# kamalmostafa/minimodem

Hardware: NVIDIA B200
Metric: audio Msamples/s demodulated (batched streams) (higher is better)
Workload: dtype f32

## Files before the change

### minimodem_b200/csrc/fsk_b200_device.cuh

```cuda
#ifndef FSK_B200_DEVICE_CUH
#define FSK_B200_DEVICE_CUH

#include <cuda_runtime.h>
#include <stdint.h>

#include "fsk_b200_internal.h"

#define FSK_FLT_EPSILON 1.1920928955078125e-07f
#define ACC_BLOCK 64u
#define FAST_MAX_N 2048u


__device__ __forceinline__ bool decide_bit(float mag_mark, float mag_space, unsigned expect,
	float2 *slot)
{
    const bool one = mag_mark > mag_space;
    const float sig = one ? mag_mark : mag_space;
    const float noise = one ? mag_space : mag_mark;
    *slot = make_float2(sig, one ? -noise : noise);
    return expect != 2u && expect != (one ? 1u : 0u);
}

__device__ __forceinline__ bool needs_resum(float mag_mark, float mag_space)
{
// ... 162 lines not shown
    }
    return best_c;
}

template <int G, class Src>
__device__ __forceinline__ float find_frame(const Src &src, unsigned base,
	const fsk_b200_geom &geo, int sel, const float4 *__restrict__ tw, float2 *scr,
	unsigned g, unsigned gmask, unsigned try_first, unsigned try_max, unsigned try_step,
	float limit, unsigned long long &best_bits, float &best_a, unsigned &best_t)
{
    return search_frames([&](unsigned t, unsigned long long &bits, float &a) {
	return frame_analyze<G, Src>(src, base + t, geo, sel, tw, scr, g, gmask, bits, a);
    }, try_first, try_max, try_step, limit, best_bits, best_a, best_t);
}


struct Ring {
    unsigned ring_s;
    unsigned R, pad;
};

__device__ __forceinline__ unsigned ring_wrap(unsigned off, unsigned R) { return off >= R ? off - R : off; }

#ifndef FSK_EMU
__device__ __forceinline__ float fast_sqrt(float x)
{
    float r;
    asm("sqrt.approx.ftz.f32 %0, %1;" : "=f"(r) : "f"(x));
    return r;
}
__device__ __forceinline__ float fast_div(float a, float b)
{
    float r;
    asm("div.approx.ftz.f32 %0, %1, %2;" : "=f"(r) : "f"(a), "f"(b));
    return r;
}
#endif

template <int G>
__device__ __forceinline__ float group_sum(float v, unsigned gmask)
{
#pragma unroll
    for (int o = G >> 1; o; o >>= 1)
	v += __shfl_xor_sync(gmask, v, o);
    return v;
}
// ... 6 lines not shown
    return v;
}
template <int G>
__device__ __forceinline__ unsigned group_add(unsigned v, unsigned gmask)
{
#pragma unroll
    for (int o = G >> 1; o; o >>= 1)
	v += __shfl_xor_sync(gmask, v, o);
    return v;
}

#ifndef FSK_EMU
__device__ __forceinline__ void cp_async_commit() { asm volatile("cp.async.commit_group;\n" ::: "memory"); }
template <int NKEEP>
__device__ __forceinline__ void cp_async_wait() { asm volatile("cp.async.wait_group %0;\n" :: "n"(NKEEP) : "memory"); }
#endif

template <int W>
struct LaneWin {
    unsigned beg[W];
    unsigned own;
    unsigned exp;
    unsigned a_end;
};

#ifndef FSK_STAGE_J
#define FSK_STAGE_J 99
#endif

template <int G, int W, int L>
__device__ __forceinline__ LaneWin<W> lane_windows(const fsk_b200_geom &geo, unsigned g)
{
    constexpr unsigned WPP = G / L;
    const unsigned part = g % L, wslot = g / L;
    LaneWin<W> lw;
    lw.own = 0;
    lw.exp = 0;
    {
	const unsigned na = min((unsigned)FSK_STAGE_J * WPP, geo.n_bits);
	lw.a_end = geo.bit_begin[na - 1u] + geo.bit_nsamples;
    }
#pragma unroll
    for (int j = 0; j < W; j++) {
	const unsigned w = j * WPP + wslot;
	const bool valid = w < geo.n_bits;
	lw.beg[j] = valid ? geo.bit_begin[w] : 0u;
	if (valid && part == (unsigned)(j % L))
	    lw.own |= 1u << j;
	const unsigned e0 = valid ? geo.expect[0][w] : 2u, e1 = valid ? geo.expect[1][w] : 2u;
	lw.exp |= (e0 << (2 * j)) | (e1 << (2 * (j + W)));
    }
    return lw;
}

template <int J0, int J1, int W, int L>
__device__ __forceinline__ void corr_pass(float (&acc)[W][4], const float *const (&p)[W],
	const float4 *tw, unsigned part, unsigned N)
{
#if defined(FSK_UNROLL) && FSK_UNROLL == 8
    _Pragma("unroll 8")
#elif defined(FSK_UNROLL) && FSK_UNROLL == 2
    _Pragma("unroll 2")
#else
    _Pragma("unroll 4")
#endif
    for (unsigned n = part; n < N; n += L) {
	const float4 c = tw[n];
#pragma unroll
	for (int j = J0; j < J1; j++) {
	    const float x = p[j][n];
	    acc[j][0] = fmaf(x, c.x, acc[j][0]);
	    acc[j][1] = fmaf(x, c.y, acc[j][1]);
	    acc[j][2] = fmaf(x, c.z, acc[j][2]);
	    acc[j][3] = fmaf(x, c.w, acc[j][3]);
	}
    }
}

struct Found {
    float confidence, amplitude;
    unsigned start, bits_lo, bits_hi;
};

template <int G, int W, int L, bool WS, bool CONSEC>
__device__ __forceinline__ float frame_finish(float (&acc)[W][4], const float *const (&p)[W],
	const unsigned own_mask, const unsigned exp_bits, const fsk_b200_geom &geo, const float4 *tw, int sel,
	unsigned g, unsigned gmask_in, unsigned &bits_lo_out, unsigned &bits_hi_out, float &ampl_out,
	float2 *bit_mags = nullptr)
{
    const unsigned gmask = WS ? 0xffffffffu : gmask_in;
    constexpr unsigned WPP = G / L;
    const unsigned N = geo.bit_nsamples, nb = geo.n_bits;
    const unsigned part = g % L, wslot = g / L;
    constexpr int KW = (W + L - 1) / L;
#ifdef FSK_NO_XCHG
    constexpr bool XCHG = false;
#else
    constexpr bool XCHG = (L == 2);
#endif
    float ax[KW][4];
    if (XCHG) {
#pragma unroll
	for (int k = 0; k < KW; k++) {
	    const int j0 = 2 * k, j1 = 2 * k + 1;
#pragma unroll
	    for (int c = 0; c < 4; c++) {
		if (j1 < W) {
		    const float send = part ? acc[j0][c] : acc[j1][c];
// ... 5 lines not shown
	}
    } else if (L > 1) {
#pragma unroll
	for (int o = L >> 1; o; o >>= 1) {
#pragma unroll
	    for (int j = 0; j < W; j++) {
#pragma unroll
		for (int k = 0; k < 4; k++)
		    acc[j][k] += __shfl_xor_sync(gmask, acc[j][k], o);
	    }
	}
    }

    const float eps_u = geo.eps_unscaled;
    float tn = 0.f, am = 0.f, as = 0.f;
    unsigned nm = 0, blo = 0, bhi = 0;
    float sig[KW];
    bool one[KW], own[KW];
    bool mismatch = false;
#pragma unroll
    for (int k = 0; k < KW; k++) {
	const unsigned jsel = part + (unsigned)(k * L);
	float a0 = 0.f, a1 = 0.f, a2 = 0.f, a3 = 0.f;
	const float *q = p[0];
#pragma unroll
	for (int pp = 0; pp < L; pp++) {
	    const int j = pp + k * L;
	    if (j < W && part == (unsigned)pp) {
		if (!XCHG) {
		    a0 = acc[j][0]; a1 = acc[j][1]; a2 = acc[j][2]; a3 = acc[j][3];
		}
		q = p[j];
	    }
	}
	if (XCHG) {
	    a0 = ax[k][0]; a1 = ax[k][1]; a2 = ax[k][2]; a3 = ax[k][3];
	}
	own[k] = (own_mask >> jsel) & 1u;
	sig[k] = 0.f;
	one[k] = false;
	if (own[k]) {
	    float mag_mark = fast_sqrt(a0 * a0 + a1 * a1);
	    float mag_space = fast_sqrt(a2 * a2 + a3 * a3);
	    const float mag_hi = fmaxf(mag_mark, mag_space);
	    if (mag_hi != 0.f && fminf(mag_mark, mag_space) < eps_u + 2e-6f * mag_hi) {
		double drm = 0., dim = 0., drs = 0., dis = 0.;
#pragma unroll 1
		for (unsigned i = 0; i < N; i++) {
		    const double x = (double)q[i];
		    const float4 c = tw[i];
		    drm = fma(x, (double)c.x, drm);
		    dim = fma(x, (double)c.y, dim);
		    drs = fma(x, (double)c.z, drs);
		    dis = fma(x, (double)c.w, dis);
		}
		const float frm = (float)drm, fim = (float)dim, frs = (float)drs, fis = (float)dis;
		mag_mark = sqrtf(frm * frm + fim * fim);
		mag_space = sqrtf(frs * frs + fis * fis);
	    }
	    const unsigned w = CONSEC ? wslot * (unsigned)W + jsel : jsel * WPP + wslot;
	    one[k] = mag_mark > mag_space;
	    sig[k] = one[k] ? mag_mark : mag_space;
	    const float noise = one[k] ? mag_space : mag_mark;
	    const unsigned e = (exp_bits >> (2u * (jsel + (sel ? (unsigned)W : 0u)))) & 3u;
	    mismatch |= e != 2u && e != (one[k] ? 1u : 0u);
	    if (bit_mags)
		bit_mags[w] = make_float2(sig[k] * geo.mag_scalar, noise * geo.mag_scalar);
	    if (noise > eps_u)
		tn += noise;
	    if (one[k]) {
		am += sig[k];
		nm++;
// ... 41 lines not shown
    float dv = 0.f;
#pragma unroll
    for (int k = 0; k < KW; k++) {
	if (own[k]) {
	    const float other = one[k] ? am : as;
	    dv += fast_div(fabsf(sig[k] - other), other);
	}
    }
    float divergence = group_sum<G>(dv, gmask);
    divergence *= 2.f;
    divergence = divergence * geo.inv_n_bits;

    if (WS && rejected) {
	bits_lo_out = bits_hi_out = 0;
	ampl_out = 0.f;
	return 0.f;
    }
    bits_lo_out = blo;
    bits_hi_out = bhi;
    ampl_out = avg_bit_sig;
    return snr * (1.0f - divergence);
}

template <int G, int W, int L, bool WS = false, bool CONSEC = false, class LW = LaneWin<W> >
__device__ __forceinline__ float frame_analyze_fast(const Ring rg, unsigned cand_off,
	const fsk_b200_geom &geo, const LW &lw, int sel, unsigned tw_s,
	unsigned g, unsigned gmask_in, unsigned &bits_lo_out, unsigned &bits_hi_out, float &ampl_out,
	int avail, bool &pending, float2 *bit_mags = nullptr)
{
    const unsigned gmask = WS ? 0xffffffffu : gmask_in;
    const float *ring = static_cast<const float *>(__cvta_shared_to_generic(rg.ring_s));
    const float4 *tw = static_cast<const float4 *>(__cvta_shared_to_generic(tw_s));
    constexpr unsigned WPP = G / L;
    const unsigned N = geo.bit_nsamples, nb = geo.n_bits, R = rg.R;
    const unsigned part = g % L, wslot = g / L;

    const float *p[W];
#pragma unroll
    for (int j = 0; j < W; j++)
	p[j] = ring + ring_wrap(cand_off + lw.beg[j], R);

    float acc[W][4];
#pragma unroll
    for (int j = 0; j < W; j++)
	acc[j][0] = acc[j][1] = acc[j][2] = acc[j][3] = 0.f;

    constexpr int SJ = (FSK_STAGE_J < W) ? FSK_STAGE_J : 0;
    if (SJ > 0) {
	if (pending && (int)lw.a_end > avail) {
	    cp_async_wait<0>();
	    __syncwarp(gmask);
	    pending = false;
	}
	corr_pass<0, SJ, W, L>(acc, p, tw, part, N);
    }
    if (pending) {
	cp_async_wait<0>();
	__syncwarp(gmask);
	pending = false;
    }
    corr_pass<SJ, W, W, L>(acc, p, tw, part, N);
    return frame_finish<G, W, L, WS, CONSEC>(acc, p, lw.own, lw.exp, geo, tw, sel, g, gmask_in, bits_lo_out,
	    bits_hi_out, ampl_out, bit_mags);
}

template <int G, int W, int L>
__device__ __noinline__ Found find_frame_ws(const Ring rg, unsigned pos_off,
	const fsk_b200_geom &geo, const LaneWin<W> lw, int sel, unsigned tw_s, unsigned g,
	unsigned gmask, bool on, unsigned try_first, unsigned try_max, unsigned try_step, float limit)
{
    Found best = { 0.f, 0.f, 0u, 0u, 0u };
    bool searching = on, nopend = false;
    for (int j = 0; __any_sync(0xffffffffu, searching); j++) {
	const int up = (j & 1) ? 1 : -1;
	const int t = (int)try_first + up * ((j + 1) / 2) * (int)try_step;
	if (t >= (int)try_max)
	    searching = false;
	const bool eval = searching && t >= 0;
	unsigned lo, hi;
	float a;
	const float c = frame_analyze_fast<G, W, L, true>(rg, eval ? ring_wrap(pos_off + (unsigned)t, rg.R) : 0u,
		geo, lw, sel, tw_s, g, gmask, lo, hi, a, 0, nopend);
	if (eval && best.confidence < c) {
	    best = Found{ c, a, (unsigned)t, lo, hi };
	    if (c >= limit)
		searching = false;
	}
    }
    return best;
}

template <int G, int W, int L>
__device__ __forceinline__ Found find_frame_fast_body(const Ring rg, unsigned pos_off,
	const fsk_b200_geom &geo, const LaneWin<W> lw, int sel, unsigned tw_s,
	unsigned g, unsigned gmask, unsigned try_first, unsigned try_max, unsigned try_step, float limit,
	int ready, bool pending, unsigned &ncand)
{
    Found best = { 0.f, 0.f, 0u, 0u, 0u };
    for (int j = 0;; j++) {
	const int up = (j & 1) ? 1 : -1;
	const int t = (int)try_first + up * ((j + 1) / 2) * (int)try_step;
	if (t >= (int)try_max)
	    break;
	if (t < 0)
	    continue;
	unsigned lo, hi;
	float a;
	ncand++;
	const float c = frame_analyze_fast<G, W, L>(rg, ring_wrap(pos_off + (unsigned)t, rg.R), geo, lw, sel,
		tw_s, g, gmask, lo, hi, a, ready - t, pending);
	if (best.confidence < c) {
	    best = Found{ c, a, (unsigned)t, lo, hi };
	    if (c >= limit)
		break;
	}
    }
    return best;
}

template <int G, int W, int L>
__device__ __forceinline__ Found find_frame_slide(const Ring rg, unsigned pos_off,
	const fsk_b200_geom &geo, const LaneWin<W> &lw, int sel, unsigned tw_s, unsigned g, unsigned gmask,
	unsigned try_first, unsigned try_max, unsigned step, unsigned &ncand)
{
    const float *ring = static_cast<const float *>(__cvta_shared_to_generic(rg.ring_s));
    const float4 *tw = static_cast<const float4 *>(__cvta_shared_to_generic(tw_s));
    const unsigned N = geo.bit_nsamples, R = rg.R;
    const unsigned part = g % L;
    const unsigned k_up = (try_max - 1u - try_first) / step;
    const unsigned k_dn = min(try_first / step, k_up);
    unsigned t = try_first - k_dn * step;
    const unsigned ncands = k_dn + k_up + 1u;

    const float *p[W];
    float acc[W][4];
#pragma unroll
    for (int j = 0; j < W; j++) {
	p[j] = ring + ring_wrap(ring_wrap(pos_off + t, R) + lw.beg[j], R);
	acc[j][0] = acc[j][1] = acc[j][2] = acc[j][3] = 0.f;
    }
    corr_pass<0, W, W, L>(acc, p, tw + t, part, N);

    Found best = { 0.f, 0.f, 0u, 0u, 0u };
    unsigned best_order = 0;
#pragma unroll 1
    for (unsigned i = 0;; i++) {
	ncand++;
	float wsum[W][4];
#pragma unroll
	for (int j = 0; j < W; j++)
#pragma unroll
	    for (int k = 0; k < 4; k++)
		wsum[j][k] = acc[j][k];
	unsigned lo, hi;
	float a;
	const float c = frame_finish<G, W, L, false, false>(wsum, p, lw.own, lw.exp, geo, tw, sel, g, gmask, lo, hi, a);
	const unsigned order = t >= try_first ? (t == try_first ? 0u : 2u * ((t - try_first) / step) - 1u)
	    : 2u * ((try_first - t) / step);
	if (best.confidence < c || (best.confidence == c && c > 0.f && order < best_order)) {
	    best = Found{ c, a, t, lo, hi };
	    best_order = order;
	}
	if (i + 1u == ncands)
	    break;
	const unsigned base = ring_wrap(pos_off + t, R);
	const float *pr[W], *pa[W];
#pragma unroll
	for (int j = 0; j < W; j++) {
	    const unsigned w0 = ring_wrap(base + lw.beg[j], R);
	    pr[j] = ring + w0;
	    pa[j] = ring + ring_wrap(w0 + N, R);
	}
	const float4 *twr = tw + t, *twa = tw + t + N;
#pragma unroll 2
	for (unsigned n = part; n < step; n += L) {
	    const float4 cr = twr[n], ca = twa[n];
#pragma unroll
	    for (int j = 0; j < W; j++) {
		const float xr = pr[j][n], xa = pa[j][n];
		acc[j][0] = fmaf(xa, ca.x, fmaf(-xr, cr.x, acc[j][0]));
		acc[j][1] = fmaf(xa, ca.y, fmaf(-xr, cr.y, acc[j][1]));
		acc[j][2] = fmaf(xa, ca.z, fmaf(-xr, cr.z, acc[j][2]));
		acc[j][3] = fmaf(xa, ca.w, fmaf(-xr, cr.w, acc[j][3]));
	    }
	}
	t += step;
#pragma unroll
	for (int j = 0; j < W; j++)
	    p[j] = ring + ring_wrap(ring_wrap(pos_off + t, R) + lw.beg[j], R);
    }
    return best;
}

template <int G, int W, int L>
__device__ __noinline__ Found find_frame_fast(const Ring rg, unsigned pos_off,
	const fsk_b200_geom &geo, const LaneWin<W> lw, int sel, unsigned tw_s,
	unsigned g, unsigned gmask, unsigned try_first, unsigned try_max, unsigned try_step, float limit,
	int ready = 0, bool pending = false)
{
    unsigned ncand = 0;
    return find_frame_fast_body<G, W, L>(rg, pos_off, geo, lw, sel, tw_s, g, gmask, try_first, try_max,
	    try_step, limit, ready, pending, ncand);
}

template <int W>
struct LaneWinM {
    unsigned beg[W];
    unsigned own;
    unsigned exp;
    unsigned wrapj;
    unsigned a_end;
    unsigned rot0;
};

template <int G, int W, int L>
__device__ __forceinline__ LaneWinM<W> lane_windows_multi(const fsk_b200_geom &geo, unsigned g)
{
    constexpr unsigned SLOTS = (unsigned)(W * (G / L));
    const unsigned part = g % L, slot = g / L;
    LaneWinM<W> lw;
    lw.own = 0;
    lw.exp = 0;
    lw.wrapj = W;
    lw.a_end = 0;
#pragma unroll
    for (int j = 0; j < W; j++) {
	const unsigned m = slot * W + j;
	const bool window = m < geo.n_bits, period = m <= geo.n_bits;
	lw.beg[j] = period ? geo.bit_nsamples * m : 0u;
	if (window && part == (unsigned)(j % L))
	    lw.own |= 1u << j;
	const unsigned e0 = window ? geo.expect[0][m] : 2u, e1 = window ? geo.expect[1][m] : 2u;
	lw.exp |= (e0 << (2 * j)) | (e1 << (2 * (j + W)));
	if (m == SLOTS - 1u)
	    lw.wrapj = j;
    }
    {
	constexpr unsigned SPG = (unsigned)(G / L);
	const unsigned stride = (geo.bit_nsamples * (unsigned)W) & 31u;
	bool collide = false;
	for (unsigned a = 0; a < SPG; a++)
	    for (unsigned b = a + 1; b < SPG; b++) {
		const unsigned d = ((b - a) * stride) & 31u;
		collide |= d < (unsigned)L || 32u - d < (unsigned)L;
	    }
	lw.rot0 = collide ? (slot | 0x80000000u) : 0u;
    }
// ... 142 lines not shown
			const float h0 = j + 1 < W ? hd[j + 1 < W ? j + 1 : 0][0] : nx[0];
			const float h1 = j + 1 < W ? hd[j + 1 < W ? j + 1 : 0][1] : nx[1];
			const float h2 = j + 1 < W ? hd[j + 1 < W ? j + 1 : 0][2] : nx[2];
			const float h3 = j + 1 < W ? hd[j + 1 < W ? j + 1 : 0][3] : nx[3];
			wp[j][0] = tl[j][0]; wp[j][1] = tl[j][1]; wp[j][2] = tl[j][2]; wp[j][3] = tl[j][3];
			rot_add(wp[j][0], wp[j][1], h0, h1, geo.rot[0], geo.rot[1]);
			rot_add(wp[j][2], wp[j][3], h2, h3, geo.rot[2], geo.rot[3]);
		    }
		} else {
		    float pv[4];
#pragma unroll
		    for (int k = 0; k < 4; k++)
			pv[k] = __shfl_sync(gmask, tl[W - 1][k], (g + G - L) & (G - 1), G);
#pragma unroll
		    for (int j = 0; j < W; j++) {
#pragma unroll
			for (int k = 0; k < 4; k++)
			    wp[j][k] = j > 0 ? tl[j > 0 ? j - 1 : 0][k] : pv[k];
			rot_add(wp[j][0], wp[j][1], hd[j][0], hd[j][1], geo.rot[0], geo.rot[1]);
			rot_add(wp[j][2], wp[j][3], hd[j][2], hd[j][3], geo.rot[2], geo.rot[3]);
		    }
		}
	    }
	    const float *q[W];
	    const unsigned cand_off = ring_wrap(pos_off + t, R);
#pragma unroll
	    for (int j = 0; j < W; j++)
		q[j] = ring + ring_wrap(cand_off + lw.beg[j], R);
	    unsigned lo, hi;
	    float a;
	    const float c = frame_finish<G, W, L, false, true>(wp, q, lw.own, lw.exp, geo, tw, sel, g, gmask,
		    lo, hi, a);
	    const unsigned order = mb.order[i];
	    if (best.confidence < c || (best.confidence == c && c > 0.f && order < best_order)) {
		best = Found{ c, a, t, lo, hi };
		best_order = order;
		if (c >= limit && kind.nbatch == 1u)
		    return FoundN{ best, ncand };
	    }
	}
    }
    return FoundN{ best, ncand };
}

struct PfxLane {
    unsigned cslot;
    unsigned kk;
    unsigned sbase;
    unsigned bb;
    unsigned peer;
    unsigned exp;
    unsigned idx0;
    bool win;
};
// ... 413 lines not shown
#define RING_BLOCK FSK_RING_BLOCK
#else
#define RING_BLOCK 128u
#endif

template <int G>
__device__ __forceinline__ void ring_block(const Ring rg, unsigned ring_s, unsigned foff,
	const float *__restrict__ src, unsigned g)
{
    constexpr int CPL = (int)(RING_BLOCK / 4u) / G;
    const unsigned d = ring_s + (foff + 4u * g) * 4u;
    const float *sp = src + 4u * g;
#pragma unroll
    for (int k = 0; k < CPL; k++)
	ldgsts16(d + (unsigned)k * 16u * G, sp + k * 4 * G);
    if (foff < rg.pad) {
#pragma unroll
	for (int k = 0; k < CPL; k++)
	    if (foff + 4u * (g + (unsigned)k * G) < rg.pad)
		ldgsts16(d + rg.R * 4u + (unsigned)k * 16u * G, sp + k * 4 * G);
    }
}

template <int G>
__device__ __forceinline__ void ring_block_at(unsigned dst, const float *__restrict__ src,
	unsigned mlim, unsigned R)
{
    constexpr int CPL = (int)(RING_BLOCK / 4u) / G;
#pragma unroll
    for (int k = 0; k < CPL; k++)
	ldgsts16(dst + (unsigned)k * 16u * G, src + k * 4 * G);
    if (dst < mlim) {
#pragma unroll
	for (int k = 0; k < CPL; k++)
	    if (dst + (unsigned)k * 16u * G < mlim)
		ldgsts16(dst + R * 4u + (unsigned)k * 16u * G, src + k * 4 * G);
    }
}

template <int G>
__device__ __forceinline__ void ring_block_tail(const Ring rg, unsigned ring_s, unsigned foff,
	const float *__restrict__ x, unsigned n, unsigned first, unsigned g)
{
    constexpr int CPL = (int)(RING_BLOCK / 4u) / G;
#pragma unroll
    for (int k = 0; k < CPL; k++) {
	const unsigned c = 4u * (g + (unsigned)k * G);
	const unsigned i = first + c;
	const unsigned valid = i + 4u <= n ? 16u : (i < n ? (n - i) * 4u : 0u);
	const float *sp = valid ? x + i : x;
	ldgsts16_zfill(ring_s + (foff + c) * 4u, sp, valid);
	if (foff + c < rg.pad)
	    ldgsts16_zfill(ring_s + (rg.R + foff + c) * 4u, sp, valid);
    }
}


__device__ __forceinline__ unsigned smem_u32(const void *p) { return (unsigned)__cvta_generic_to_shared(p); }

#ifndef FSK_EMU
__device__ __forceinline__ void mbar_init(unsigned bar, unsigned count)
{
    asm volatile("mbarrier.init.shared::cta.b64 [%0], %1;\n" :: "r"(bar), "r"(count) : "memory");
}
__device__ __forceinline__ void mbar_fence_init()
{
    asm volatile("fence.mbarrier_init.release.cluster;\n" ::: "memory");
    asm volatile("fence.proxy.async.shared::cta;\n" ::: "memory");
}
__device__ __forceinline__ void mbar_arrive_expect_tx(unsigned bar, unsigned bytes)
{
    asm volatile("mbarrier.arrive.expect_tx.shared::cta.b64 _, [%0], %1;\n" :: "r"(bar), "r"(bytes) : "memory");
}
__device__ __forceinline__ bool mbar_try_wait(unsigned bar, unsigned parity)
{
    unsigned ok;
// ... 150 lines not shown
```

### minimodem_b200/csrc/fsk_b200_internal.h

```cpp
#ifndef FSK_B200_INTERNAL_H
#define FSK_B200_INTERNAL_H

#include "fsk_b200.h"

#ifdef __cplusplus
extern "C" {
#endif

typedef struct fsk_b200_geom {
    unsigned int n_bits;
    unsigned int bit_nsamples;
    unsigned int span;
    unsigned int lanes_per_window;
    float	mag_scalar;
    float	eps_unscaled;
    float	inv_n_bits;
    unsigned int tw_entries;
    float	rot[4];
    unsigned int bit_begin[FSK_B200_MAX_BITS];
    unsigned char expect[2][FSK_B200_MAX_BITS];
} fsk_b200_geom;

struct fsk_b200_loopc;
typedef struct fsk_b200_loopc {
    unsigned int frame_nsamples, expect_nsamples, nsamples_overscan;
    unsigned int try_max_nocarrier, try_max_carrier;
    float	confidence_threshold, confidence_search_limit;
    unsigned int slide;
} fsk_b200_loopc;

#define FSK_MULTI_MAXB 4
typedef struct fsk_b200_mbatch {
    uint16_t	anchor;
    uint16_t	rho1, rho2;
    uint16_t	t[3];
    uint8_t	ncand;
    uint8_t	csplit;
    uint8_t	cseg[3];
    int8_t	shift[3];
    uint8_t	order[3];
    uint8_t	pad;
// ... 89 lines not shown
```

### minimodem_b200/csrc/fsk_b200_kernels.cu

```cuda
#include <cuda_runtime.h>
#include <errno.h>
#include <math.h>
#include <stdint.h>
#include <stdio.h>
#include <stdlib.h>
#include <string.h>

#include "fsk_b200_internal.h"
#include "fsk_b200_device.cuh"
#include "fsk_b200_decode_core.h"

static unsigned long long g_launches;

#ifndef FSK_EMU
#define FSK_LAUNCH(kernel, grid, block, smem, stream, ...) kernel<<<(grid), (block), (smem), (stream)>>>(__VA_ARGS__)
#define FSK_DYN_SMEM(name) extern __shared__ float4 name[]
#endif

#define CUDA_TRY(call) do { cudaError_t e_ = (call); if (e_ != cudaSuccess) { \
    fsk_b200_set_error("%s: %s", #call, cudaGetErrorString(e_)); return -EIO; } } while (0)


struct Smem {
    const float4 *tw;
    float *ring;
    float2 *scr;
    unsigned long long *bars;
    float4 *pre, *tot;
    const float4 *loc;
    float4 *red;
};

template <int G>
__device__ __forceinline__ Smem carve(float4 *smem, const fsk_b200_geom &geo,
	const float4 *__restrict__ tw_global, unsigned tw_in_smem, unsigned ring_floats, unsigned pad,
	unsigned pfx_chunks = 0, const float *pfx_loc = nullptr, unsigned pfx_red = 0)
{
    const unsigned N = geo.tw_entries, wpb = blockDim.x >> 5;
    Smem s;
    float4 *p = smem;
    if (tw_in_smem) {
	for (unsigned i = threadIdx.x; i < N; i += blockDim.x)
	    p[i] = tw_global[i];
	s.tw = p;
	p += N;
    } else {
	s.tw = tw_global;
    }
    const unsigned spw = 32 / G;
    const unsigned slot = (threadIdx.x >> 5) * spw + (threadIdx.x & 31) / G;
    float *rings = reinterpret_cast<float *>(p);
    if (!ring_floats)
	pad = 0u;
    s.ring = rings + (size_t)slot * (ring_floats + pad);
    float2 *scrs = reinterpret_cast<float2 *>(rings + (size_t)wpb * spw * (ring_floats + pad));
    s.scr = scrs + (size_t)slot * geo.n_bits;
    unsigned long long *bars = reinterpret_cast<unsigned long long *>(scrs + (((size_t)wpb * spw * geo.n_bits + 1u) & ~(size_t)1u));
    s.bars = bars + 2 * slot;
    float4 *pfx = reinterpret_cast<float4 *>(bars + 2 * (size_t)wpb * spw);
    s.loc = pfx;
    if (pfx_chunks) {
	if (threadIdx.x < 32u)
	    reinterpret_cast<float *>(pfx)[threadIdx.x] = pfx_loc[threadIdx.x];
	pfx += 8;
    }
    s.pre = pfx + (size_t)slot * (pfx_chunks + 32u + pfx_red);
    s.tot = s.pre + pfx_chunks;
    s.red = s.tot + 32u;
    __syncthreads();
    return s;
}

#define GROUP_VARS \
    const unsigned lane = threadIdx.x & 31, g = lane % G, sidx = lane / G, spw = 32 / G; \
    const unsigned gmask = (G == 32) ? 0xffffffffu : (((1u << G) - 1u) << (sidx * G)); \
    const unsigned wpb = blockDim.x >> 5, warp = threadIdx.x >> 5; \
    (void)lane
// ... 96 lines not shown
#else
#define EARLY_REQ 1
#endif
#ifndef FSK_MINBLOCKS
#define FSK_MINBLOCKS 4
#endif
#ifndef FSK_MAXTHREADS
#define FSK_MAXTHREADS 128
#endif
#ifndef FSK_PFX_MAXTHREADS
#define FSK_PFX_MAXTHREADS 512
#endif
template <int G, int W, int L, int MODE, int FILL, int SRC = 0>
__global__ void __launch_bounds__(MODE == 3 ? FSK_PFX_MAXTHREADS : FSK_MAXTHREADS,
	MODE == 3 ? 1 : (MODE == 2 && G >= 16) ? 3 : FSK_MINBLOCKS)
k_rx(const __grid_constant__ fsk_b200_geom geo, const __grid_constant__ fsk_b200_loopc lc,
	const float4 *__restrict__ tw_global, unsigned tw_in_smem, unsigned ring_floats,
	unsigned lookahead, const __grid_constant__ RxArgs a, const __grid_constant__ fsk_b200_mplan mp,
	const float4 *__restrict__ tw_sample, const __grid_constant__ fsk_b200_pfx pg)
{
    FSK_DYN_SMEM(smem4);
    const unsigned ring_pad = MODE == 3 ? 4u * pg.S + 8u : (geo.bit_nsamples + 3u) & ~3u;
    constexpr int LB = W == 1 ? 0 : W;
    const Smem sm = carve<G>(smem4, geo, tw_global, tw_in_smem, ring_floats, ring_pad, MODE == 3 ? 32u * pg.tstride : 0u,
	    &pg.loc[0][0][0], (MODE == 3 && LB == 0) ? 32u : 0u);
    GROUP_VARS;
    const Ring rg = { smem_u32(sm.ring), ring_floats, ring_pad };
    const unsigned tw_s = tw_in_smem ? smem_u32(sm.tw) : 0u;
    const LaneWin<W> lw = lane_windows<G, W, L>(geo, g);
    const LaneWinM<W> lwm = lane_windows_multi<G, W, L>(geo, g);
    const PfxLane pfl = MODE == 3 ? pfx_lane(geo, pg, lane) : PfxLane();
    const unsigned pre_s = smem_u32(sm.pre), tot_s = smem_u32(sm.tot), loc_s = smem_u32(sm.loc), red_s = smem_u32(sm.red);
    const unsigned R = ring_floats;

    for (unsigned s = (blockIdx.x * wpb + warp) * spw + sidx; s < a.nstreams;
	    s += gridDim.x * wpb * spw) {
	fsk_b200_stream_state st = a.states[s];
	if (st.done)
	    continue;
	const float *x = SRC ? (const float *)nullptr : a.samples + (size_t)s * a.stride;
	const int16_t *x16 = SRC ? a.samples16 + (size_t)s * a.stride : (const int16_t *)nullptr;
	const unsigned n = (unsigned)min((size_t)(a.nsamples ? a.nsamples[s] : a.nsamples_all), a.stride);
	fsk_b200_frame *out = a.frames + (size_t)s * a.max_frames;
	constexpr unsigned AL = SRC ? 7u : 3u;

	unsigned pos = (unsigned)st.pos;
	unsigned nframes = st.nframes;
	unsigned carrier = st.carrier, noconfidence = st.noconfidence;
	float track_amplitude = st.track_amplitude, peak_confidence = st.peak_confidence;
	unsigned long long carrier_nsamples = st.carrier_nsamples;
	float confidence_total = st.confidence_total, amplitude_total = st.amplitude_total;
	unsigned nframes_decoded = st.nframes_decoded;
	unsigned done = 0;
	unsigned ncand = 0, nsearch = 0;
	bool mhint = st.reserved != 0u;

	unsigned pos_off = pos & AL;
	unsigned filled = pos & ~AL;
	unsigned conv = filled, coff = 0;
	const unsigned need_max = lc.try_max_nocarrier - 1u + geo.span;
	const unsigned n4 = (n + 3u) & ~3u;
	const unsigned bar0 = smem_u32(sm.bars), bar1 = bar0 + 8u;
	unsigned kphase = 0;
	bool tail_fix = false;

	const unsigned ring_s = rg.ring_s;
	unsigned landed = pos & ~AL;
	const unsigned dst0 = ring_s + 16u * g, dst_end = dst0 + R * 4u;
	const unsigned mlim = ring_s + rg.pad * 4u;
	unsigned fdst = dst0;
	const float *fsrc = SRC ? x : x + filled + 4u * g;
	auto request_at = [&](unsigned to, unsigned base) {
	    const unsigned lim = min(to, (base & ~AL) + R - (RING_BLOCK - 1u));
	    while (filled < lim) {
		if (SRC) {
		    if (filled + RING_BLOCK <= n)
			ring_block16<G>(ring_s, (fdst - dst0) >> 2, x16 + filled, g);
		    else
			ring_block16_tail<G>(ring_s, (fdst - dst0) >> 2, x16, n, filled, g);
		} else if (filled + RING_BLOCK <= n)
		    ring_block_at<G>(fdst, fsrc, mlim, R);
		else
		    ring_block_tail<G>(rg, ring_s, (fdst - dst0) >> 2, x, n, filled, g);
		filled += RING_BLOCK;
		fsrc += RING_BLOCK;
		fdst += RING_BLOCK * 4u;
		if (fdst == dst_end)
		    fdst = dst0;
	    }
	    cp_async_commit();
	};
	auto request = [&](unsigned to) {
	    if (FILL == 0) {
		request_at(to, pos);
	    } else {
		const unsigned to_b = min(to, n4);
		const unsigned from_b = min(filled, to_b);
		if (g == 0)
		    ring_issue_bulk(rg, x, pos, pos_off, from_b, to_b, (kphase & 1u) ? bar1 : bar0);
		if (n < n4 && from_b < n4 && to_b == n4 && to_b > from_b)
		    tail_fix = true;
		kphase++;
		if (to > max(filled, n4))
		    ring_zero<G>(rg, pos, pos_off, max(filled, n4), to, g);
		if (to > filled)
		    filled = to;
	    }
	};
	auto settle = [&](bool all) {
// ... 137 lines not shown
			    float am;
			    const float c = frame_analyze_fast<G, W, L, false, true, LaneWinM<W> >(rg,
				    ring_wrap(pos_off + try_first, R), geo, lwm, which, tw_s, g, gmask, lo, hi, am,
				    ready - (int)try_first, pending);
			    ncand++;
			    if (0.f < c) {
				seed = Found{ c, am, try_first, lo, hi };
				decided = c >= limit;
			    }
			    skip = 1;
			    mhint = !decided;
			}
			if (decided)
			    f = seed;
			else {
			    const FoundN r = find_frame_multi<G, W, L>(rg, pos_off, geo, lwm, which, tw_s, g, gmask,
				    kind, limit, pending, seed, skip);
			    f = r.f;
			    ncand += r.ncand;
			    if (pass == 0 && !skip)
				mhint = r.ncand > 1u;
			}
		    } else if (MODE == 0 && FILL != 3 && pass == 1 && lc.slide)
			f = find_frame_slide<G, W, L>(rg, pos_off, geo, lw, which, tw_s, g, gmask, try_first, try_max,
				step, ncand);
		    else
			f = find_frame_fast_body<G, W, L>(rg, pos_off, geo, lw, which, tw_s, g,
				gmask, try_first, try_max, step, limit, ready, pending, ncand);
		    if (pass) {
			refined = f;
			break;
		    }
		    first = f;
		    float c = f.confidence;
		    const bool below_peak = c < peak_confidence * 0.75f;
		    if (f.amplitude < track_amplitude * 0.25f)
			c = 0.f;
		    if (!(c > lc.confidence_threshold) || !(below_peak || !carrier) || !(c < INFINITY)
			    || try_step <= 1u)
			break;
		    step = try_max / 8u;
		    if (step == 0)
			step = 1;
		    limit = INFINITY;
		    which = 0;
		    pending = false;
		}
		confidence = first.confidence;
		amplitude = first.amplitude;
		frame_start = first.start;
// ... 838 lines not shown
    return best != ~0u;
}

static bool split_for(int G, unsigned n_bits, int force_L, int *W, int *L)
{
    double best = -1.0;
    for (int l = 1; l <= 4 && l <= G; l *= 2) {
	if (force_L && l != force_L)
	    continue;
	const unsigned wpp = (unsigned)(G / l);
	const unsigned w = (n_bits + wpp - 1) / wpp;
	if (w > 4 || !fast_combo(G, (int)w, l))
	    continue;
	const double util = (double)n_bits / (double)(w * wpp);
	if (util >= best - 1e-9) {
	    best = util;
	    *W = (int)w;
	    *L = l;
	}
    }
    return best > 0.0;
}

static int pick_shape(const CudaEngine *ce, const fsk_b200_geom *g, unsigned need_floats,
	unsigned max_advance, size_t nstreams, Shape *sh, const fsk_b200_loopc *lc = NULL)
{
    sh->geo = *g;
    memset(&sh->mplan, 0, sizeof(sh->mplan));
    const size_t smem_max = (size_t)ce->smem_optin;
    const size_t tw_bytes = (size_t)g->bit_nsamples * sizeof(float4);
    sh->tw_in_smem = tw_bytes <= 24 * 1024;
    const size_t fixed = sh->tw_in_smem ? tw_bytes : 0;
    const size_t pad_bytes = (size_t)((g->bit_nsamples + 3u) & ~3u) * 4;
    const size_t scr_bytes = (size_t)g->n_bits * sizeof(float2) + pad_bytes + 16;

    const unsigned ring_min = (need_floats + 8u + 2u * RING_BLOCK - 1u) / RING_BLOCK * RING_BLOCK;
    (void)max_advance;
    unsigned ring = ce->ring ? ((unsigned)ce->ring + RING_BLOCK - 1u) / RING_BLOCK * RING_BLOCK : ring_min;
    if (ring < ring_min)
	ring = ring_min;
    if (!ce->ring) {
	while (ring > ring_min && (smem_max - fixed) / ((size_t)ring * 4 + scr_bytes) < 24)
	    ring -= RING_BLOCK;
    }

    int G = ce->lanes;
// ... 157 lines not shown
	}
    }
    sh->geo.tw_entries = sh->mode == 3 ? sh->pfx_tw_stage : g->bit_nsamples;
    sh->slide = 0;
    if (sh->mode == 0 && lc && lc->slide && g->tw_entries > g->bit_nsamples && sh->tw_in_smem) {
	const size_t extra = (size_t)(g->tw_entries - g->bit_nsamples) * sizeof(float4);
	if (sh->smem + extra <= smem_max) {
	    sh->smem += extra;
	    sh->geo.tw_entries = g->tw_entries;
	    sh->slide = 1;
	}
    }
    sh->G = G;
    sh->W = W;
    sh->L = L;
    sh->wpb = wpb;
    sh->ring = ring;
    {
	const unsigned base_need = need_floats + 8u + RING_BLOCK;
	const unsigned slack = ring > base_need ? ring - base_need : 0u;
	sh->lookahead = slack < max_advance ? slack : max_advance;
    }
    sh->geo.lanes_per_window = (unsigned)L;
    const size_t streams_per_block = (size_t)wpb * (32 / G);
    size_t blocks = (nstreams + streams_per_block - 1) / streams_per_block;
    if (blocks > 0x7fffffff)
	blocks = 0x7fffffff;
    sh->blocks = (int)(blocks ? blocks : 1);
    return 0;
}

template <int G, int W, int L, int MODE>
static cudaError_t launch_find_t(const Shape &sh, const CudaEngine *ce, const FindArgs &a, cudaStream_t st)
{
    cudaError_t e = cudaFuncSetAttribute(k_find_frame<G, W, L, MODE>,
	    cudaFuncAttributeMaxDynamicSharedMemorySize, (int)sh.smem);
    if (e != cudaSuccess)
	return e;
    FSK_LAUNCH((k_find_frame<G, W, L, MODE>), sh.blocks, sh.wpb * 32, sh.smem, st, sh.geo, ce->d_tw,
	    sh.tw_in_smem, sh.ring, a);
    g_launches++;
    return cudaGetLastError();
}

extern "C" int fsk_b200_cuda_find_frame_batch(void *p, const fsk_b200_geom *g, const float *samples,
	size_t nstreams, size_t stride, const uint32_t *offset, const uint32_t *nvalid,
// ... 485 lines not shown
```

Measured before the change: 1.153 million.

## Interleave per-stream rings in shared memory and rotate correlation walk to avoid bank conflicts

For the G=8 mode-0 direct-fill path, the four stream rings of a warp are interleaved in 16-byte chunks (column stride CS) instead of being laid out contiguously, with ring indexing via ring_at. The correlation loop is also restructured: each lane window can start its sample walk at a rotated offset (chosen on the host by a bank-conflict cost model in walk_policy), running a common unrolled segment and then a wrapped remainder. Both changes target shared-memory bank conflicts during the per-bit correlation. In exchange they add index arithmetic, a second remainder loop, and more template variants.

```diff
diff --git a/minimodem_b200/csrc/fsk_b200_device.cuh b/minimodem_b200/csrc/fsk_b200_device.cuh
--- a/minimodem_b200/csrc/fsk_b200_device.cuh
+++ b/minimodem_b200/csrc/fsk_b200_device.cuh
@@ -208,6 +208,9 @@
 
 __device__ __forceinline__ unsigned ring_wrap(unsigned off, unsigned R) { return off >= R ? off - R : off; }
 
+template <int CS>
+__device__ __forceinline__ unsigned ring_at(unsigned t) { return CS == 1 ? t : (t & ~3u) * (unsigned)CS + (t & 3u); }
+
 #ifndef FSK_EMU
 __device__ __forceinline__ float fast_sqrt(float x)
 {
@@ -260,10 +263,15 @@
     unsigned own;
     unsigned exp;
     unsigned a_end;
+    unsigned rot;
+    unsigned ncommon;
 };
 
 #ifndef FSK_STAGE_J
 #define FSK_STAGE_J 99
+#endif
+#ifndef FSK_UNROLL
+#define FSK_UNROLL 4
 #endif
 
 template <int G, int W, int L>
@@ -278,6 +286,8 @@
 	const unsigned na = min((unsigned)FSK_STAGE_J * WPP, geo.n_bits);
 	lw.a_end = geo.bit_begin[na - 1u] + geo.bit_nsamples;
     }
+    lw.rot = geo.walk ? wslot : 0u;
+    lw.ncommon = geo.bit_nsamples / (unsigned)L - (geo.walk ? WPP - 1u : 0u);
 #pragma unroll
     for (int j = 0; j < W; j++) {
 	const unsigned w = j * WPP + wslot;
@@ -291,27 +301,64 @@
     return lw;
 }
 
-template <int J0, int J1, int W, int L>
-__device__ __forceinline__ void corr_pass(float (&acc)[W][4], const float *const (&p)[W],
-	const float4 *tw, unsigned part, unsigned N)
-{
-#if defined(FSK_UNROLL) && FSK_UNROLL == 8
-    _Pragma("unroll 8")
-#elif defined(FSK_UNROLL) && FSK_UNROLL == 2
-    _Pragma("unroll 2")
-#else
-    _Pragma("unroll 4")
-#endif
-    for (unsigned n = part; n < N; n += L) {
-	const float4 c = tw[n];
+template <int J0, int J1, int W, int L, int CS>
+__device__ __forceinline__ void corr_pass(float (&acc)[W][4], const float *ring, const unsigned (&s0)[W],
+	const float4 *tw, unsigned part, unsigned N, unsigned rot, unsigned ncommon)
+{
+    auto step = [&](const float4 c, const float (&x)[W]) {
 #pragma unroll
 	for (int j = J0; j < J1; j++) {
-	    const float x = p[j][n];
-	    acc[j][0] = fmaf(x, c.x, acc[j][0]);
-	    acc[j][1] = fmaf(x, c.y, acc[j][1]);
-	    acc[j][2] = fmaf(x, c.z, acc[j][2]);
-	    acc[j][3] = fmaf(x, c.w, acc[j][3]);
-	}
+	    acc[j][0] = fmaf(x[j], c.x, acc[j][0]);
+	    acc[j][1] = fmaf(x[j], c.y, acc[j][1]);
+	    acc[j][2] = fmaf(x[j], c.z, acc[j][2]);
+	    acc[j][3] = fmaf(x[j], c.w, acc[j][3]);
+	}
+    };
+    const unsigned n_a = part + (unsigned)L * rot;
+    const float4 *tp = tw + n_a;
+    constexpr int P = CS == 1 ? 1 : (L % 4 == 0 ? 1 : (L % 2 == 0 ? 2 : 4));
+    constexpr unsigned PSTRIDE = (unsigned)(CS * L * P);
+    const float *q[W][P];
+#pragma unroll
+    for (int j = J0; j < J1; j++)
+#pragma unroll
+	for (int i = 0; i < P; i++)
+	    q[j][i] = ring + ring_at<CS>(s0[j] + n_a + (unsigned)(L * i));
+    const unsigned nu = ncommon / (unsigned)P;
+    constexpr int UNR = FSK_UNROLL / P;
+#pragma unroll (UNR)
+    for (unsigned u = 0; u < nu; u++) {
+#pragma unroll
+	for (int i = 0; i < P; i++) {
+	    float x[W];
+#pragma unroll
+	    for (int j = J0; j < J1; j++)
+		x[j] = q[j][i][PSTRIDE * u];
+	    step(tp[(unsigned)L * ((unsigned)P * u + (unsigned)i)], x);
+	}
+    }
+#pragma unroll
+    for (int i = 0; i < P - 1; i++) {
+	if ((unsigned)i < ncommon % (unsigned)P) {
+	    float x[W];
+#pragma unroll
+	    for (int j = J0; j < J1; j++)
+		x[j] = q[j][i][PSTRIDE * nu];
+	    step(tp[(unsigned)L * ((unsigned)P * nu + (unsigned)i)], x);
+	}
+    }
+    const unsigned K = (N - part + (unsigned)L - 1u) / (unsigned)L;
+#pragma unroll 1
+    for (unsigned k = ncommon; k < K; k++) {
+	unsigned kk = rot + k;
+	if (kk >= K)
+	    kk -= K;
+	const unsigned n = part + (unsigned)L * kk;
+	float x[W];
+#pragma unroll
+	for (int j = J0; j < J1; j++)
+	    x[j] = ring[ring_at<CS>(s0[j] + n)];
+	step(tw[n], x);
     }
 }
 
@@ -320,8 +367,8 @@
     unsigned start, bits_lo, bits_hi;
 };
 
-template <int G, int W, int L, bool WS, bool CONSEC>
-__device__ __forceinline__ float frame_finish(float (&acc)[W][4], const float *const (&p)[W],
+template <int G, int W, int L, bool WS, bool CONSEC, int CS = 1>
+__device__ __forceinline__ float frame_finish(float (&acc)[W][4], const float *ring, const unsigned (&s0)[W],
 	const unsigned own_mask, const unsigned exp_bits, const fsk_b200_geom &geo, const float4 *tw, int sel,
 	unsigned g, unsigned gmask_in, unsigned &bits_lo_out, unsigned &bits_hi_out, float &ampl_out,
 	float2 *bit_mags = nullptr)
@@ -373,7 +420,7 @@
     for (int k = 0; k < KW; k++) {
 	const unsigned jsel = part + (unsigned)(k * L);
 	float a0 = 0.f, a1 = 0.f, a2 = 0.f, a3 = 0.f;
-	const float *q = p[0];
+	unsigned q = s0[0];
 #pragma unroll
 	for (int pp = 0; pp < L; pp++) {
 	    const int j = pp + k * L;
@@ -381,7 +428,7 @@
 		if (!XCHG) {
 		    a0 = acc[j][0]; a1 = acc[j][1]; a2 = acc[j][2]; a3 = acc[j][3];
 		}
-		q = p[j];
+		q = s0[j];
 	    }
 	}
 	if (XCHG) {
@@ -398,7 +445,7 @@
 		double drm = 0., dim = 0., drs = 0., dis = 0.;
 #pragma unroll 1
 		for (unsigned i = 0; i < N; i++) {
-		    const double x = (double)q[i];
+		    const double x = (double)ring[ring_at<CS>(q + i)];
 		    const float4 c = tw[i];
 		    drm = fma(x, (double)c.x, drm);
 		    dim = fma(x, (double)c.y, dim);
@@ -486,7 +533,7 @@
     return snr * (1.0f - divergence);
 }
 
-template <int G, int W, int L, bool WS = false, bool CONSEC = false, class LW = LaneWin<W> >
+template <int G, int W, int L, bool WS = false, bool CONSEC = false, class LW = LaneWin<W>, int CS = 1>
 __device__ __forceinline__ float frame_analyze_fast(const Ring rg, unsigned cand_off,
 	const fsk_b200_geom &geo, const LW &lw, int sel, unsigned tw_s,
 	unsigned g, unsigned gmask_in, unsigned &bits_lo_out, unsigned &bits_hi_out, float &ampl_out,
@@ -499,10 +546,10 @@
     const unsigned N = geo.bit_nsamples, nb = geo.n_bits, R = rg.R;
     const unsigned part = g % L, wslot = g / L;
 
-    const float *p[W];
+    unsigned s0[W];
 #pragma unroll
     for (int j = 0; j < W; j++)
-	p[j] = ring + ring_wrap(cand_off + lw.beg[j], R);
+	s0[j] = ring_wrap(cand_off + lw.beg[j], R);
 
     float acc[W][4];
 #pragma unroll
@@ -516,15 +563,15 @@
 	    __syncwarp(gmask);
 	    pending = false;
 	}
-	corr_pass<0, SJ, W, L>(acc, p, tw, part, N);
+	corr_pass<0, SJ, W, L, CS>(acc, ring, s0, tw, part, N, lw.rot, lw.ncommon);
     }
     if (pending) {
 	cp_async_wait<0>();
 	__syncwarp(gmask);
 	pending = false;
     }
-    corr_pass<SJ, W, W, L>(acc, p, tw, part, N);
-    return frame_finish<G, W, L, WS, CONSEC>(acc, p, lw.own, lw.exp, geo, tw, sel, g, gmask_in, bits_lo_out,
+    corr_pass<SJ, W, W, L, CS>(acc, ring, s0, tw, part, N, lw.rot, lw.ncommon);
+    return frame_finish<G, W, L, WS, CONSEC, CS>(acc, ring, s0, lw.own, lw.exp, geo, tw, sel, g, gmask_in, bits_lo_out,
 	    bits_hi_out, ampl_out, bit_mags);
 }
 
@@ -554,7 +601,7 @@
     return best;
 }
 
-template <int G, int W, int L>
+template <int G, int W, int L, int CS = 1>
 __device__ __forceinline__ Found find_frame_fast_body(const Ring rg, unsigned pos_off,
 	const fsk_b200_geom &geo, const LaneWin<W> lw, int sel, unsigned tw_s,
 	unsigned g, unsigned gmask, unsigned try_first, unsigned try_max, unsigned try_step, float limit,
@@ -571,7 +618,8 @@
 	unsigned lo, hi;
 	float a;
 	ncand++;
-	const float c = frame_analyze_fast<G, W, L>(rg, ring_wrap(pos_off + (unsigned)t, rg.R), geo, lw, sel,
+	const float c = frame_analyze_fast<G, W, L, false, false, LaneWin<W>, CS>(rg, ring_wrap(pos_off + (unsigned)t, rg.R),
+		geo, lw, sel,
 		tw_s, g, gmask, lo, hi, a, ready - t, pending);
 	if (best.confidence < c) {
 	    best = Found{ c, a, (unsigned)t, lo, hi };
@@ -582,7 +630,7 @@
     return best;
 }
 
-template <int G, int W, int L>
+template <int G, int W, int L, int CS = 1>
 __device__ __forceinline__ Found find_frame_slide(const Ring rg, unsigned pos_off,
 	const fsk_b200_geom &geo, const LaneWin<W> &lw, int sel, unsigned tw_s, unsigned g, unsigned gmask,
 	unsigned try_first, unsigned try_max, unsigned step, unsigned &ncand)
@@ -596,14 +644,14 @@
     unsigned t = try_first - k_dn * step;
     const unsigned ncands = k_dn + k_up + 1u;
 
-    const float *p[W];
+    unsigned s0[W];
     float acc[W][4];
 #pragma unroll
     for (int j = 0; j < W; j++) {
-	p[j] = ring + ring_wrap(ring_wrap(pos_off + t, R) + lw.beg[j], R);
+	s0[j] = ring_wrap(ring_wrap(pos_off + t, R) + lw.beg[j], R);
 	acc[j][0] = acc[j][1] = acc[j][2] = acc[j][3] = 0.f;
     }
-    corr_pass<0, W, W, L>(acc, p, tw + t, part, N);
+    corr_pass<0, W, W, L, CS>(acc, ring, s0, tw + t, part, N, lw.rot, lw.ncommon);
 
     Found best = { 0.f, 0.f, 0u, 0u, 0u };
     unsigned best_order = 0;
@@ -618,7 +666,7 @@
 		wsum[j][k] = acc[j][k];
 	unsigned lo, hi;
 	float a;
-	const float c = frame_finish<G, W, L, false, false>(wsum, p, lw.own, lw.exp, geo, tw, sel, g, gmask, lo, hi, a);
+	const float c = frame_finish<G, W, L, false, false, CS>(wsum, ring, s0, lw.own, lw.exp, geo, tw, sel, g, gmask, lo, hi, a);
 	const unsigned order = t >= try_first ? (t == try_first ? 0u : 2u * ((t - try_first) / step) - 1u)
 	    : 2u * ((try_first - t) / step);
 	if (best.confidence < c || (best.confidence == c && c > 0.f && order < best_order)) {
@@ -628,12 +676,12 @@
 	if (i + 1u == ncands)
 	    break;
 	const unsigned base = ring_wrap(pos_off + t, R);
-	const float *pr[W], *pa[W];
+	unsigned sr[W], sa[W];
 #pragma unroll
 	for (int j = 0; j < W; j++) {
 	    const unsigned w0 = ring_wrap(base + lw.beg[j], R);
-	    pr[j] = ring + w0;
-	    pa[j] = ring + ring_wrap(w0 + N, R);
+	    sr[j] = w0;
+	    sa[j] = ring_wrap(w0 + N, R);
 	}
 	const float4 *twr = tw + t, *twa = tw + t + N;
 #pragma unroll 2
@@ -641,7 +689,7 @@
 	    const float4 cr = twr[n], ca = twa[n];
 #pragma unroll
 	    for (int j = 0; j < W; j++) {
-		const float xr = pr[j][n], xa = pa[j][n];
+		const float xr = ring[ring_at<CS>(sr[j] + n)], xa = ring[ring_at<CS>(sa[j] + n)];
 		acc[j][0] = fmaf(xa, ca.x, fmaf(-xr, cr.x, acc[j][0]));
 		acc[j][1] = fmaf(xa, ca.y, fmaf(-xr, cr.y, acc[j][1]));
 		acc[j][2] = fmaf(xa, ca.z, fmaf(-xr, cr.z, acc[j][2]));
@@ -651,7 +699,7 @@
 	t += step;
 #pragma unroll
 	for (int j = 0; j < W; j++)
-	    p[j] = ring + ring_wrap(ring_wrap(pos_off + t, R) + lw.beg[j], R);
+	    s0[j] = ring_wrap(ring_wrap(pos_off + t, R) + lw.beg[j], R);
     }
     return best;
 }
@@ -674,6 +722,7 @@
     unsigned exp;
     unsigned wrapj;
     unsigned a_end;
+    unsigned rot, ncommon;
     unsigned rot0;
 };
 
@@ -687,6 +736,8 @@
     lw.exp = 0;
     lw.wrapj = W;
     lw.a_end = 0;
+    lw.rot = 0;
+    lw.ncommon = geo.bit_nsamples / (unsigned)L;
 #pragma unroll
     for (int j = 0; j < W; j++) {
 	const unsigned m = slot * W + j;
@@ -875,14 +926,14 @@
 		    }
 		}
 	    }
-	    const float *q[W];
+	    unsigned q[W];
 	    const unsigned cand_off = ring_wrap(pos_off + t, R);
 #pragma unroll
 	    for (int j = 0; j < W; j++)
-		q[j] = ring + ring_wrap(cand_off + lw.beg[j], R);
+		q[j] = ring_wrap(cand_off + lw.beg[j], R);
 	    unsigned lo, hi;
 	    float a;
-	    const float c = frame_finish<G, W, L, false, true>(wp, q, lw.own, lw.exp, geo, tw, sel, g, gmask,
+	    const float c = frame_finish<G, W, L, false, true>(wp, ring, q, lw.own, lw.exp, geo, tw, sel, g, gmask,
 		    lo, hi, a);
 	    const unsigned order = mb.order[i];
 	    if (best.confidence < c || (best.confidence == c && c > 0.f && order < best_order)) {
@@ -1342,23 +1393,24 @@
     }
 }
 
-template <int G>
+template <int G, int CS = 1>
 __device__ __forceinline__ void ring_block_at(unsigned dst, const float *__restrict__ src,
 	unsigned mlim, unsigned R)
 {
     constexpr int CPL = (int)(RING_BLOCK / 4u) / G;
+    constexpr unsigned DS = 16u * G * CS;
 #pragma unroll
     for (int k = 0; k < CPL; k++)
-	ldgsts16(dst + (unsigned)k * 16u * G, src + k * 4 * G);
+	ldgsts16(dst + (unsigned)k * DS, src + k * 4 * G);
     if (dst < mlim) {
 #pragma unroll
 	for (int k = 0; k < CPL; k++)
-	    if (dst + (unsigned)k * 16u * G < mlim)
-		ldgsts16(dst + R * 4u + (unsigned)k * 16u * G, src + k * 4 * G);
-    }
-}
-
-template <int G>
+	    if (dst + (unsigned)k * DS < mlim)
+		ldgsts16(dst + R * 4u * CS + (unsigned)k * DS, src + k * 4 * G);
+    }
+}
+
+template <int G, int CS = 1>
 __device__ __forceinline__ void ring_block_tail(const Ring rg, unsigned ring_s, unsigned foff,
 	const float *__restrict__ x, unsigned n, unsigned first, unsigned g)
 {
@@ -1369,9 +1421,9 @@
 	const unsigned i = first + c;
 	const unsigned valid = i + 4u <= n ? 16u : (i < n ? (n - i) * 4u : 0u);
 	const float *sp = valid ? x + i : x;
-	ldgsts16_zfill(ring_s + (foff + c) * 4u, sp, valid);
+	ldgsts16_zfill(ring_s + ring_at<CS>(foff + c) * 4u, sp, valid);
 	if (foff + c < rg.pad)
-	    ldgsts16_zfill(ring_s + (rg.R + foff + c) * 4u, sp, valid);
+	    ldgsts16_zfill(ring_s + ring_at<CS>(rg.R + foff + c) * 4u, sp, valid);
     }
 }
 
diff --git a/minimodem_b200/csrc/fsk_b200_internal.h b/minimodem_b200/csrc/fsk_b200_internal.h
--- a/minimodem_b200/csrc/fsk_b200_internal.h
+++ b/minimodem_b200/csrc/fsk_b200_internal.h
@@ -17,6 +17,7 @@
     float	inv_n_bits;
     unsigned int tw_entries;
     float	rot[4];
+    unsigned int walk;
     unsigned int bit_begin[FSK_B200_MAX_BITS];
     unsigned char expect[2][FSK_B200_MAX_BITS];
 } fsk_b200_geom;
diff --git a/minimodem_b200/csrc/fsk_b200_kernels.cu b/minimodem_b200/csrc/fsk_b200_kernels.cu
--- a/minimodem_b200/csrc/fsk_b200_kernels.cu
+++ b/minimodem_b200/csrc/fsk_b200_kernels.cu
@@ -31,7 +31,7 @@
     float4 *red;
 };
 
-template <int G>
+template <int G, int CS = 1>
 __device__ __forceinline__ Smem carve(float4 *smem, const fsk_b200_geom &geo,
 	const float4 *__restrict__ tw_global, unsigned tw_in_smem, unsigned ring_floats, unsigned pad,
 	unsigned pfx_chunks = 0, const float *pfx_loc = nullptr, unsigned pfx_red = 0)
@@ -52,7 +52,10 @@
     float *rings = reinterpret_cast<float *>(p);
     if (!ring_floats)
 	pad = 0u;
-    s.ring = rings + (size_t)slot * (ring_floats + pad);
+    if (CS == 1)
+	s.ring = rings + (size_t)slot * (ring_floats + pad);
+    else
+	s.ring = rings + (size_t)(slot - slot % spw) * (ring_floats + pad) + 4u * (slot % spw);
     float2 *scrs = reinterpret_cast<float2 *>(rings + (size_t)wpb * spw * (ring_floats + pad));
     s.scr = scrs + (size_t)slot * geo.n_bits;
     unsigned long long *bars = reinterpret_cast<unsigned long long *>(scrs + (((size_t)wpb * spw * geo.n_bits + 1u) & ~(size_t)1u));
@@ -195,7 +198,11 @@
     FSK_DYN_SMEM(smem4);
     const unsigned ring_pad = MODE == 3 ? 4u * pg.S + 8u : (geo.bit_nsamples + 3u) & ~3u;
     constexpr int LB = W == 1 ? 0 : W;
-    const Smem sm = carve<G>(smem4, geo, tw_global, tw_in_smem, ring_floats, ring_pad, MODE == 3 ? 32u * pg.tstride : 0u,
+#ifndef FSK_TMP_CS
+#define FSK_TMP_CS 4
+#endif
+    constexpr int CS = (MODE == 0 && FILL == 0 && SRC == 0 && G == 8) ? FSK_TMP_CS : 1;
+    const Smem sm = carve<G, CS>(smem4, geo, tw_global, tw_in_smem, ring_floats, ring_pad, MODE == 3 ? 32u * pg.tstride : 0u,
 	    &pg.loc[0][0][0], (MODE == 3 && LB == 0) ? 32u : 0u);
     GROUP_VARS;
     const Ring rg = { smem_u32(sm.ring), ring_floats, ring_pad };
@@ -239,8 +246,8 @@
 
 	const unsigned ring_s = rg.ring_s;
 	unsigned landed = pos & ~AL;
-	const unsigned dst0 = ring_s + 16u * g, dst_end = dst0 + R * 4u;
-	const unsigned mlim = ring_s + rg.pad * 4u;
+	const unsigned dst0 = ring_s + 16u * CS * g, dst_end = dst0 + R * 4u * CS;
+	const unsigned mlim = ring_s + rg.pad * 4u * CS;
 	unsigned fdst = dst0;
 	const float *fsrc = SRC ? x : x + filled + 4u * g;
 	auto request_at = [&](unsigned to, unsigned base) {
@@ -252,12 +259,12 @@
 		    else
 			ring_block16_tail<G>(ring_s, (fdst - dst0) >> 2, x16, n, filled, g);
 		} else if (filled + RING_BLOCK <= n)
-		    ring_block_at<G>(fdst, fsrc, mlim, R);
+		    ring_block_at<G, CS>(fdst, fsrc, mlim, R);
 		else
-		    ring_block_tail<G>(rg, ring_s, (fdst - dst0) >> 2, x, n, filled, g);
+		    ring_block_tail<G, CS>(rg, ring_s, (fdst - dst0) / (4u * CS), x, n, filled, g);
 		filled += RING_BLOCK;
 		fsrc += RING_BLOCK;
-		fdst += RING_BLOCK * 4u;
+		fdst += RING_BLOCK * 4u * CS;
 		if (fdst == dst_end)
 		    fdst = dst0;
 	    }
@@ -441,10 +448,10 @@
 				mhint = r.ncand > 1u;
 			}
 		    } else if (MODE == 0 && FILL != 3 && pass == 1 && lc.slide)
-			f = find_frame_slide<G, W, L>(rg, pos_off, geo, lw, which, tw_s, g, gmask, try_first, try_max,
+			f = find_frame_slide<G, W, L, CS>(rg, pos_off, geo, lw, which, tw_s, g, gmask, try_first, try_max,
 				step, ncand);
 		    else
-			f = find_frame_fast_body<G, W, L>(rg, pos_off, geo, lw, which, tw_s, g,
+			f = find_frame_fast_body<G, W, L, CS>(rg, pos_off, geo, lw, which, tw_s, g,
 				gmask, try_first, try_max, step, limit, ready, pending, ncand);
 		    if (pass) {
 			refined = f;
@@ -1329,6 +1336,31 @@
     return best > 0.0;
 }
 
+static bool walk_policy(int mode, int G, int W, int L, const fsk_b200_geom *g)
+{
+    const unsigned WPP = (unsigned)(G / L), N = g->bit_nsamples;
+    if (mode != 0 || G != 8 || N / (unsigned)L < WPP)
+	return false;
+#ifdef FSK_TMP_WALK_OFF
+    return false;
+#endif
+    unsigned long cost[2] = { 0, 0 };
+    for (unsigned r = 0; r < 2; r++)
+	for (unsigned c = 0; c < 8; c++)
+	    for (unsigned j = 0; j < (unsigned)W; j++)
+		for (unsigned k = 0; k + WPP - 1u < N / (unsigned)L; k++) {
+		    unsigned cnt[8] = { 0 }, mx = 0;
+		    for (unsigned q = 0; q < WPP && j * WPP + q < g->n_bits; q++)
+			for (unsigned p = 0; p < (unsigned)L; p++) {
+			    const unsigned t = c + g->bit_begin[j * WPP + q] + p + (unsigned)L * ((r ? q : 0u) + k);
+			    if (++cnt[t & 7u] > mx)
+				mx = cnt[t & 7u];
+			}
+		    cost[r] += mx;
+		}
+    return cost[1] < cost[0];
+}
+
 static int pick_shape(const CudaEngine *ce, const fsk_b200_geom *g, unsigned need_floats,
 	unsigned max_advance, size_t nstreams, Shape *sh, const fsk_b200_loopc *lc = NULL)
 {
@@ -1532,6 +1564,7 @@
 	sh->lookahead = slack < max_advance ? slack : max_advance;
     }
     sh->geo.lanes_per_window = (unsigned)L;
+    sh->geo.walk = walk_policy(sh->mode, G, W, L, g) ? 1u : 0u;
     const size_t streams_per_block = (size_t)wpb * (32 / G);
     size_t blocks = (nstreams + streams_per_block - 1) / streams_per_block;
     if (blocks > 0x7fffffff)
```

After: 835,100, median of 6. -27.6%, worse.
